# Chang-Tun-Yu/HLS-final-Visual-Odometry

Hardware: AMD Instinct MI355X
Metric: stereo frame-pairs/sec (detect+match), KITTI 1241x376; matches bit-exact (higher is better)
Workload: dtype u8; 1 GPU; KITTI 1241x376 stereo quad-match (prev/curr x L/R), default 50x50 bins; noise=0, gpu_max_hw_queues=4, streams_per_gpu=256, frames_in_hbm=8, parallelism=1x independent stream groups

## Files before the change

hls-final-visual-odometry_amd/csrc/kernels_detect.hip:

```cpp
#include "vh_dev.h"
#include "vh_wave.h"
#include <type_traits>

namespace {

__global__ void half_res_kernel(VhImages src, uint8_t *__restrict__ dst, VhGeom g) {
  const int32_t id = blockIdx.z;
  const uint8_t *__restrict__ I = vh_image_ptr(src, id);
  uint8_t *__restrict__ O = dst + (int64_t)id * g.bplm * g.Hm;
  const int32_t u = blockIdx.x * blockDim.x + threadIdx.x;
  const int32_t v = blockIdx.y;
  if (u >= g.bplm) return;
  uint32_t val = 0;
  if (u < g.Wm) {
    const int64_t r0 = (int64_t)(2 * v) * g.bpl + 2 * u, r1 = r0 + g.bpl;
    val = ((uint32_t)I[r0] + I[r0 + 1] + I[r1] + I[r1 + 1]) >> 2;
  }
  O[(int64_t)v * g.bplm + u] = (uint8_t)val;
}

__global__ void __launch_bounds__(256)
detect_nms_kernel(VhImages im, VhGeom g, uint64_t *__restrict__ rec, int32_t *__restrict__ chunk_count) {
  extern __shared__ __attribute__((aligned(16))) uint8_t smem[];
  uint8_t *sI = smem;
  int16_t *sF1 = (int16_t *)(smem + (size_t)g.IH * g.IWp);
  int16_t *sF2 = sF1 + (size_t)g.FH * g.FWp;

  const int32_t id = blockIdx.z;
  const uint8_t *__restrict__ I = vh_image_ptr(im, id);
  const int32_t n = g.n, n1 = n + 1;
  const int32_t bx0 = blockIdx.x * g.tbx, by0 = blockIdx.y * g.tby;
  const int32_t fx0 = VH_MARGIN + bx0 * n1, fy0 = VH_MARGIN + by0 * n1;
  const int32_t ix0 = fx0 - 2, iy0 = fy0 - 2;
  const int32_t tid = threadIdx.x;

  for (int32_t k = tid; k < g.IH * g.IWp; k += 256) {
    const int32_t r = k / g.IWp, c = k - r * g.IWp;
    const int32_t gx = ix0 + c, gy = iy0 + r;
    uint8_t v = 0;
    if (c < g.IW && gx < g.bplm && gy < g.Hm) v = I[(int64_t)gy * g.bplm + gx];
    sI[k] = v;
  }
  __syncthreads();

  {
    const int32_t nseg = max(1, 256 / g.FW);
    const int32_t rows_per = (g.FH + nseg - 1) / nseg;
    for (int32_t task = tid; task < g.FW * nseg; task += 256) {
      const int32_t seg = task / g.FW, cx = task - seg * g.FW;
      const int32_t r0 = seg * rows_per, r1 = min(g.FH, r0 + rows_per);
      if (r0 >= r1) continue;
      int32_t h5[5], h3[5], hc[5], cc[5];
#pragma unroll
      for (int32_t k = 0; k < 4; k++) {
        const uint8_t *p = sI + (size_t)(r0 + k) * g.IWp + cx;
        const int32_t a = p[0], b = p[1], c = p[2], d = p[3], e = p[4];
        h5[k + 1] = a + b + c + d + e; h3[k + 1] = b + c + d; hc[k + 1] = a + b - d - e; cc[k + 1] = c;
      }
      for (int32_t fr = r0; fr < r1; fr++) {
#pragma unroll
        for (int32_t k = 0; k < 4; k++) { h5[k] = h5[k + 1]; h3[k] = h3[k + 1]; hc[k] = hc[k + 1]; cc[k] = cc[k + 1]; }
        const uint8_t *p = sI + (size_t)(fr + 4) * g.IWp + cx;
        const int32_t a = p[0], b = p[1], c = p[2], d = p[3], e = p[4];
        h5[4] = a + b + c + d + e; h3[4] = b + c + d; hc[4] = a + b - d - e; cc[4] = c;
        const int32_t f2 = hc[0] + hc[1] - hc[3] - hc[4];
        const int32_t f1 = -(h5[0] + h5[1] + h5[2] + h5[3] + h5[4]) + 2 * (h3[1] + h3[2] + h3[3]) + 7 * cc[2];
        sF1[(size_t)fr * g.FWp + cx] = (int16_t)f1;
        sF2[(size_t)fr * g.FWp + cx] = (int16_t)f2;
      }
    }
  }
  __syncthreads();

  int32_t *sCnt = (int32_t *)(sF2 + (size_t)g.FH * g.FWp);
  uint32_t *sWork = (uint32_t *)(sCnt + 1);
  uint16_t *sCode = (uint16_t *)(sWork + 4 * g.tbx * g.tby);
  const int32_t nblk_tile = g.tbx * g.tby;
  if (tid == 0) *sCnt = 0;
  for (int32_t k = tid; k < 4 * nblk_tile; k += 256) sCode[k] = VH_NO_CODE;
  __syncthreads();
  const int32_t xlim = (g.Wm - 1 - VH_MARGIN) - fx0, ylim = (g.Hm - 1 - VH_MARGIN) - fy0;
  const int32_t lby = tid / g.tbx, lbx = tid - lby * g.tbx;
  const int32_t bx = bx0 + lbx, by = by0 + lby;
  const bool have_block = tid < nblk_tile && bx < g.nbx && by < g.nby;
  if (have_block) {
    const int32_t fx = n + lbx * n1, fy = n + lby * n1;
    int32_t ex[4], ey[4], ev[4];
    ex[0] = ex[1] = ex[2] = ex[3] = fx;
    ey[0] = ey[1] = ey[2] = ey[3] = fy;
    ev[0] = ev[1] = sF1[(size_t)fy * g.FWp + fx];
    ev[2] = ev[3] = sF2[(size_t)fy * g.FWp + fx];
    for (int32_t j2 = fy; j2 <= fy + n; j2++) {
      for (int32_t i2 = fx; i2 <= fx + n; i2++) {
        int32_t cur = sF1[(size_t)j2 * g.FWp + i2];
        if (cur < ev[0]) { ex[0] = i2; ey[0] = j2; ev[0] = cur; }
        else if (cur > ev[1]) { ex[1] = i2; ey[1] = j2; ev[1] = cur; }
        cur = sF2[(size_t)j2 * g.FWp + i2];
        if (cur < ev[2]) { ex[2] = i2; ey[2] = j2; ev[2] = cur; }
        else if (cur > ev[3]) { ex[3] = i2; ey[3] = j2; ev[3] = cur; }
      }
    }
#pragma unroll
    for (int32_t c = 0; c < 4; c++) {
      const bool pass = (c & 1) ? (ev[c] >= g.tau) : (ev[c] <= -g.tau);
      if (pass) sWork[atomicAdd(sCnt, 1)] = (uint32_t)ex[c] | ((uint32_t)ey[c] << 10) | ((uint32_t)c << 20) | ((uint32_t)tid << 22);
    }
  }
  __syncthreads();
  const int32_t nwork = *sCnt;
  for (int32_t w = tid; w < nwork; w += 256) {
    const uint32_t e = sWork[w];
    const int32_t cx = e & 1023, cy = (e >> 10) & 1023, c = (e >> 20) & 3, owner = e >> 22;
    const int32_t oby = owner / g.tbx, obx = owner - oby * g.tbx;
    const int32_t fx = n + obx * n1, fy = n + oby * n1;
    const int16_t *F = (c < 2) ? sF1 : sF2;
    const bool is_min = (c & 1) == 0;
    const int32_t val = F[(size_t)cy * g.FWp + cx];
    const int32_t jhi = min(cy + n, ylim), ihi = min(cx + n, xlim);
    bool ok = true;
    for (int32_t j2 = cy - n; j2 <= jhi && ok; j2++) {
      for (int32_t i2 = cx - n; i2 <= ihi; i2++) {
        const int32_t cur = F[(size_t)j2 * g.FWp + i2];
        const bool outside = (i2 < fx) | (i2 > fx + n) | (j2 < fy) | (j2 > fy + n);
        if (outside && (is_min ? (cur < val) : (cur > val))) { ok = false; break; }
      }
    }
    if (ok) sCode[owner * 4 + c] = (uint16_t)(((cy - fy) << 6) | (cx - fx));
  }
  __syncthreads();
  if (have_block) {
    uint64_t code = 0;
    int32_t cnt = 0;
#pragma unroll
    for (int32_t c = 0; c < 4; c++) {
      const uint32_t pc = sCode[tid * 4 + c];
      code |= (uint64_t)pc << (16 * c);
      cnt += pc != VH_NO_CODE ? 1 : 0;
    }
    const int32_t blk = by * g.nbx + bx;
    rec[(int64_t)id * g.nblocks + blk] = code;
    if (cnt) atomicAdd(&chunk_count[(int64_t)id * g.nchunks + blk / VH_CHUNK], cnt);
  }
}

#ifdef VH_EMIT_TIMING
__device__ unsigned long long g_emit_t[8];
extern "C" int32_t vh_debug_emit_timing(unsigned long long *out, int32_t reset) {
  if (hipMemcpyFromSymbol(out, HIP_SYMBOL(g_emit_t), sizeof(g_emit_t)) != hipSuccess) return -3;
  if (reset) { unsigned long long z[8] = {0}; z[6] = ~0ull; if (hipMemcpyToSymbol(HIP_SYMBOL(g_emit_t), z, sizeof(z)) != hipSuccess) return -3; }
  return 0;
}
#define VH_TICK_IMPL(k) do { __syncthreads(); if (t_on_) { const unsigned long long now_ = __builtin_readcyclecounter(); atomicAdd(&g_emit_t[k], now_ - t_prev_); t_prev_ = now_; if ((k) == 4) atomicMax(&g_emit_t[7], now_); } } while (0)
#define VH_TICK_INIT_IMPL const bool t_on_ = threadIdx.x == 0 && (blockIdx.x + gridDim.x * (blockIdx.y + gridDim.y * blockIdx.z)) % 61 == 0; unsigned long long t_prev_ = __builtin_readcyclecounter(); if (t_on_) { atomicAdd(&g_emit_t[5], 1ull); atomicMin(&g_emit_t[6], t_prev_); }
#endif
#if defined(VH_EMIT_TIMING) && VH_EMIT_TIMING == 2
#define VH_DTICK(k) VH_TICK_IMPL(k)
#define VH_DTICK_INIT VH_TICK_INIT_IMPL
#else
#define VH_DTICK(k) do { } while (0)
#define VH_DTICK_INIT do { } while (0)
#endif
#if defined(VH_EMIT_TIMING) && VH_EMIT_TIMING != 2
#define VH_ETICK(k) VH_TICK_IMPL(k)
#define VH_ETICK_INIT VH_TICK_INIT_IMPL
#else
#define VH_ETICK(k) do { } while (0)
#define VH_ETICK_INIT do { } while (0)
#endif

#ifdef VH_EXP_DET_STOP
#define VH_DET_STOP(k)                                                                                   \
  if (VH_EXP_DET_STOP == (k) && g.nbx > 0) {                                                              \
    const int32_t sbx = bx0 + tid % T::TBX, sby = by0 + tid / T::TBX;                                     \
    if (sbx < g.nbx && sby < g.nby) rec[(int64_t)id * g.nblocks + sby * g.nbx + sbx] = ~0ull;              \
    return;                                                                                               \
  }
#else
#define VH_DET_STOP(k) do { } while (0)
#endif

template <int N> struct DetTile {
  static constexpr int N1 = N + 1, TBX = 32, TBY = 8;
  static constexpr int FW = TBX * N1 + 2 * N, FH = TBY * N1 + 2 * N;
  static constexpr int IW = FW + 4, IH = FH + 4;
  static constexpr int OFF = (VH_MARGIN - 2) & 3;
  static constexpr int DW = ((IW + 3 + 3) / 4 + 3) / 4 * 4;
  static constexpr int IP = DW * 4;
  static constexpr int NC = DW / 4;
  static constexpr int groups(int px) { return (FW + OFF + px - 1) / px; }
  static constexpr int seg_cost(int px, int s) {
    const int rows = (FH + s - 1) / s, waves = (groups(px) * s + 63) / 64;
    const int hrow = px == 4 ? 28 : 18, vrow = px == 4 ? 26 : 13;
    return groups(px) * s > 256 || rows * (s - 1) >= FH ? (1 << 30) : 1000 * ((rows + 4) * hrow + rows * vrow) + waves;
  }
  static constexpr int best_seg(int px) {
    int b = 1;
    for (int s = 2; s <= 16; s++)
      if (seg_cost(px, s) < seg_cost(px, b)) b = s;
    return b;
  }
#ifdef VH_DET_PX
  static constexpr int PX = VH_DET_PX;
  static constexpr int SEG = VH_DET_SEG;
#else
  static constexpr int PX = seg_cost(2, best_seg(2)) < seg_cost(4, best_seg(4)) ? 2 : 4;
  static constexpr int SEG = best_seg(PX);
#endif
  static constexpr int G = groups(PX);
  static constexpr int FP = PX * G;
  static constexpr int ROWS = (FH + SEG - 1) / SEG;
  static constexpr int BIAS = 8192;
  static_assert((G - 1) * PX / 4 + 1 <= DW - 1, "a group reads the staged dword it starts in and the next one");
  static_assert(G * SEG <= 256, "one lane per (group, row segment)");
  static constexpr int LAST = FH - (SEG - 1) * ROWS;
  static_assert(LAST >= 1, "every segment has rows");
};

template <int N>
__global__ void __launch_bounds__(256)
detect_nms_fast_kernel(VhImages im, VhGeom g, uint64_t *__restrict__ rec, int32_t *__restrict__ chunk_count) {
  using T = DetTile<N>;
  constexpr int N1 = T::N1, WN = 2 * N + 1;
  VH_DET_SETPRIO();
  constexpr int X_BYTES = (T::IH * T::IP > 6144) ? T::IH * T::IP : 6144;
  __shared__ __attribute__((aligned(16))) int16_t sF1[T::FH * T::FP];
  __shared__ __attribute__((aligned(16))) int16_t sF2[T::FH * T::FP];
  __shared__ __attribute__((aligned(16))) uint8_t sX[X_BYTES];
  uint8_t *sI = sX;

  const int32_t id = blockIdx.z, tid = threadIdx.x;
  const uint8_t *__restrict__ I = vh_image_ptr(im, id);
  const int32_t bx0 = blockIdx.x * T::TBX, by0 = blockIdx.y * T::TBY;
  const int32_t fx0 = VH_MARGIN + bx0 * N1, fy0 = VH_MARGIN + by0 * N1;
  const int32_t ix0 = fx0 - 2, iy0 = fy0 - 2;
  const int32_t ax0 = ix0 - T::OFF;
  VH_DTICK_INIT;

  {
    constexpr int NLD = (T::IH * T::NC + 255) / 256;
    typedef uint32_t u32x4a4 __attribute__((ext_vector_type(4), aligned(4)));
    typedef uint32_t u32x4 __attribute__((ext_vector_type(4)));
    const uint32_t last = (uint32_t)g.Hm * (uint32_t)g.bplm - 16u;
    u32x4 stg[NLD];
#pragma unroll
    for (int32_t i = 0; i < NLD; i++) {
      const int32_t k = min(tid + 256 * i, T::IH * T::NC - 1);
      const int32_t r = k / T::NC, c = k - r * T::NC;
      stg[i] = *(const u32x4a4 *)(I + min((uint32_t)(iy0 + r) * (uint32_t)g.bplm + (uint32_t)(ax0 + 16 * c), last));
    }
    __builtin_amdgcn_sched_barrier(0);
#pragma unroll
    for (int32_t i = 0; i < NLD; i++) {
      const int32_t k = tid + 256 * i;
      if (k < T::IH * T::NC) ((u32x4 *)sI)[k] = stg[i];
    }
  }
  __syncthreads();

  VH_DTICK(0);
  VH_DET_STOP(1);
  if (tid < T::G * T::SEG) {
    constexpr int PX = T::PX, NR = PX / 2;
    const int32_t seg = tid / T::G, gq = tid - seg * T::G;
    const int32_t r0 = seg * T::ROWS;
    {
      constexpr uint32_t HB = 512u * 0x00010001u, KB = (uint32_t)T::BIAS * 0x00010001u;
      const uint32_t *p = (const uint32_t *)sI + r0 * T::DW + (gq * PX) / 4;
      const uint32_t sel0 = 0x0c010c00u + ((PX == 2 && (gq & 1)) ? 0x00020002u : 0u);
      uint32_t *o1 = (uint32_t *)sF1 + (r0 * T::FP + PX * gq) / 2, *o2 = (uint32_t *)sF2 + (r0 * T::FP + PX * gq) / 2;
      uint32_t h5[NR][5], h3[NR][5], pc[NR][4], cc[NR][5], hcp[NR], S5[NR];
#pragma unroll
      for (int32_t h = 0; h < NR; h++) S5[h] = 0u;
#pragma unroll
      for (int32_t t = 0; t < T::ROWS + 4; t++) {
        if (t - 4 < T::LAST || r0 + t - 4 < T::FH) {
          const uint32_t A = p[t * T::DW], B = p[t * T::DW + 1];
          uint32_t pk[PX + 3];
#pragma unroll
          for (int32_t k = 0; k < PX + 3; k++) pk[k] = __builtin_amdgcn_perm(B, A, sel0 + (uint32_t)k * 0x00010001u);
          uint32_t n5[NR], n3[NR], nc[NR], nz[NR];
          if (PX == 4) {
            const uint32_t a01 = pk[0] + pk[1], a23 = pk[2] + pk[3], a34 = pk[3] + pk[4], a56 = pk[5] + pk[6];
            n3[0] = a23 + pk[1];             n3[NR - 1] = a34 + pk[5];
            n5[0] = n3[0] + pk[0] + pk[4];   n5[NR - 1] = n3[NR - 1] + pk[2] + pk[6];
            nc[0] = (a01 + HB) - a34;        nc[NR - 1] = (a23 + HB) - a56;
            nz[0] = pk[2];                   nz[NR - 1] = pk[4];
          } else {
            n3[0] = pk[1] + pk[2] + pk[3];
            n5[0] = n3[0] + pk[0] + pk[4];
            nc[0] = ((pk[0] + pk[1]) + HB) - (pk[3] + pk[4]);
            nz[0] = pk[2];
          }
          uint32_t f1[NR], f2[NR];
#pragma unroll
          for (int32_t h = 0; h < NR; h++) {
            const uint32_t old5 = h5[h][0];
#pragma unroll
            for (int32_t k = 0; k < 4; k++) { h5[h][k] = h5[h][k + 1]; h3[h][k] = h3[h][k + 1]; cc[h][k] = cc[h][k + 1]; }
            h5[h][4] = n5[h]; h3[h][4] = n3[h]; cc[h][4] = nz[h];
            S5[h] += n5[h];
            if (t >= 5) S5[h] -= old5;
#pragma unroll
            for (int32_t k = 0; k < 3; k++) pc[h][k] = pc[h][k + 1];
            if (t > 0) pc[h][3] = hcp[h] + nc[h];
            hcp[h] = nc[h];
            if (t >= 4) {
              const uint32_t S3 = h3[h][1] + h3[h][2] + h3[h][3];
              f2[h] = (pc[h][0] + KB) - pc[h][3];
              f1[h] = ((S3 + S3) + (__umul24(cc[h][2], 7u) + KB)) - S5[h];
            }
          }
          if (t >= 4) {
            if (PX == 4) {
              *(uint2 *)(o1 + (t - 4) * (T::FP / 2)) = make_uint2(f1[0], f1[NR - 1]);
              *(uint2 *)(o2 + (t - 4) * (T::FP / 2)) = make_uint2(f2[0], f2[NR - 1]);
            } else {
              o1[(t - 4) * (T::FP / 2)] = f1[0];
              o2[(t - 4) * (T::FP / 2)] = f2[0];
            }
          }
        }
      }
    }
  }
  __syncthreads();
  VH_DTICK(1);
  VH_DET_STOP(2);

  const int32_t xlim = min(max((g.Wm - 1 - VH_MARGIN) - fx0, 0), T::FW - 1);
  const int32_t ylim = min(max((g.Hm - 1 - VH_MARGIN) - fy0, 0), T::FH - 1);
  const int32_t lby = tid / T::TBX, lbx = tid % T::TBX;
  const int32_t bx = bx0 + lbx, by = by0 + lby;
  const bool have_block = bx < g.nbx && by < g.nby;
  const int32_t fx = N + lbx * N1, fy = N + lby * N1;
  uint32_t *sQueue = (uint32_t *)sX;
  uint16_t *sCode = (uint16_t *)(sQueue + 1024);
  __shared__ uint32_t sQueueN;
  if (tid == 0) sQueueN = 0;
  ((uint2 *)sCode)[tid] = make_uint2(VH_NO_CODE * 0x00010001u, VH_NO_CODE * 0x00010001u);
  __syncthreads();
  {
    typedef int16_t i16x2 __attribute__((ext_vector_type(2)));
    const int32_t lane = tid & 63;
    bool cand[4];
    uint32_t ext[4];
#pragma unroll
    for (int32_t plane = 0; plane < 2; plane++) {
      const int16_t *b = (plane ? sF2 : sF1) + fy * T::FP + fx + T::OFF;
      int32_t vn, vx;
      if (N & 1) {
        const i16x2 *bw = (const i16x2 *)b;
        i16x2 mn = bw[0], mx = mn;
#pragma unroll
        for (int32_t j = 0; j < N1; j++) {
#pragma unroll
          for (int32_t d = 0; d < N1 / 2; d++) {
            if (d == 0 && j == 0) continue;
            const i16x2 w = bw[j * (T::FP / 2) + d];
            mn = __builtin_elementwise_min(mn, w);
            mx = __builtin_elementwise_max(mx, w);
          }
        }
        vn = min((int32_t)mn.x, (int32_t)mn.y);
        vx = max((int32_t)mx.x, (int32_t)mx.y);
      } else {
        vn = vx = b[0];
#pragma unroll
        for (int32_t k = 1; k < N1 * N1; k++) {
          const int32_t cur = b[(k / N1) * T::FP + k % N1];
          vn = min(vn, cur);
          vx = max(vx, cur);
        }
      }
      cand[2 * plane] = have_block && vn <= T::BIAS - g.tau;
      cand[2 * plane + 1] = have_block && vx >= T::BIAS + g.tau;
      ext[2 * plane] = (uint32_t)vn;
      ext[2 * plane + 1] = (uint32_t)vx;
    }
    uint64_t bal[4];
#pragma unroll
    for (int32_t t = 0; t < 4; t++) bal[t] = __ballot(cand[t]);
    const uint32_t n0 = (uint32_t)__popcll(bal[0]), n1 = (uint32_t)__popcll(bal[1]);
    const uint32_t add = (n0 + (uint32_t)__popcll(bal[2])) | ((n1 + (uint32_t)__popcll(bal[3])) << 16);
    if (add) {
      uint32_t base = 0;
      if (lane == 0) base = atomicAdd(&sQueueN, add);
      base = __builtin_amdgcn_readfirstlane(base);
#pragma unroll
      for (int32_t t = 0; t < 4; t++) {
        const int32_t mm = t & 1;
        const uint32_t first = ((base >> (16 * mm)) & 0xFFFFu) + (t >= 2 ? (mm ? n1 : n0) : 0u);
        const uint32_t rank = (uint32_t)vh_wave_rank(bal[t]);
        if (cand[t]) sQueue[mm * 512 + first + rank] = (uint32_t)tid | ((uint32_t)t << 8) | (ext[t] << 16);
      }
    }
  }
  __syncthreads();
  VH_DTICK(2);
  VH_DET_STOP(3);
  {
    const int32_t n0 = (int32_t)(sQueueN & 0xFFFFu), ntot = n0 + (int32_t)(sQueueN >> 16);
    const bool unclipped = xlim == T::FW - 1 && ylim == T::FH - 1;
    auto check = [&](auto kind, auto no_clip, int32_t e) {
      const uint32_t q = sQueue[e < n0 ? e : 512 + e - n0];
      const int32_t owner = q & 255, type = (q >> 8) & 3;
      const int32_t ofy = N + (owner / T::TBX) * N1, ofx = N + (owner % T::TBX) * N1;
      const int16_t *F = ((type & 2) ? sF2 : sF1) + T::OFF;
      const int32_t val = (int32_t)(q >> 16);
      const int16_t *bb = F + ofy * T::FP + ofx;
      int32_t pos = (N << 6) | N;
#pragma unroll
      for (int32_t idx = N1 * N1 - 2; idx >= 0; idx--)
        pos = bb[(idx / N1) * T::FP + idx % N1] == val ? (((idx / N1) << 6) | (idx % N1)) : pos;
      const int32_t bj = pos >> 6, bi = pos & 63;
      const int32_t cy = ofy + bj, cx = ofx + bi;
      int32_t v[WN * WN];
      if (decltype(no_clip)::value) {
        const int16_t *w = F + (cy - N) * T::FP + (cx - N);
#pragma unroll
        for (int32_t j = 0; j < WN; j++)
#pragma unroll
          for (int32_t k = 0; k < WN; k++) v[j * WN + k] = w[j * T::FP + k];
      } else {
        int32_t col[WN];
#pragma unroll
        for (int32_t k = 0; k < WN; k++) col[k] = min(cx - N + k, xlim);
#pragma unroll
        for (int32_t j = 0; j < WN; j++) {
          const int16_t *row = F + min(cy - N + j, ylim) * T::FP;
#pragma unroll
          for (int32_t k = 0; k < WN; k++) v[j * WN + k] = row[col[k]];
        }
      }
      const int32_t centre = v[N * WN + N];
      int32_t emin = centre, emax = centre;
#pragma unroll
      for (int32_t k = 0; k < WN * WN; k++) {
        if (decltype(kind)::value != 1) emin = min(emin, v[k]);
        if (decltype(kind)::value != 0) emax = max(emax, v[k]);
      }
      const int32_t ext = decltype(kind)::value == 0 ? emin : decltype(kind)::value == 1 ? emax : ((type & 1) ? emax : emin);
      if (ext == centre) sCode[owner * 4 + type] = (uint16_t)((bj << 6) | bi);
    };
    typedef std::integral_constant<int, 0> KMin;
    typedef std::integral_constant<int, 1> KMax;
    typedef std::integral_constant<int, 2> KBoth;
    for (int32_t e = tid; e < ntot; e += 256) {
      const int32_t e0 = __builtin_amdgcn_readfirstlane(e & ~63);
      if (e0 + 63 < n0) { if (unclipped) check(KMin{}, std::true_type{}, e); else check(KMin{}, std::false_type{}, e); }
      else if (e0 >= n0) { if (unclipped) check(KMax{}, std::true_type{}, e); else check(KMax{}, std::false_type{}, e); }
      else { if (unclipped) check(KBoth{}, std::true_type{}, e); else check(KBoth{}, std::false_type{}, e); }
    }
  }
  __syncthreads();
  VH_DTICK(3);
  VH_DET_STOP(4);
  uint32_t codes[4];
  {
    const uint2 cw = ((const uint2 *)sCode)[tid];
    codes[0] = cw.x & 0xFFFFu; codes[1] = cw.x >> 16; codes[2] = cw.y & 0xFFFFu; codes[3] = cw.y >> 16;
  }

  __shared__ int32_t sChunk[16];
  const int32_t chunk_lo = (by0 * g.nbx + bx0) / VH_CHUNK;
  if (tid < 16) sChunk[tid] = 0;
  __syncthreads();
  if (have_block) {
    int32_t cnt = 0;
#pragma unroll
    for (int32_t c = 0; c < 4; c++) cnt += codes[c] != VH_NO_CODE ? 1 : 0;
    const int32_t blk = by * g.nbx + bx;
    rec[(int64_t)id * g.nblocks + blk] = (uint64_t)(codes[0] | (codes[1] << 16)) | ((uint64_t)(codes[2] | (codes[3] << 16)) << 32);
    if (cnt) atomicAdd(&sChunk[blk / VH_CHUNK - chunk_lo], cnt);
  }
  __syncthreads();
  if (tid < 16 && sChunk[tid]) atomicAdd(&chunk_count[(int64_t)id * g.nchunks + chunk_lo + tid], sChunk[tid]);
  VH_DTICK(4);
}

__constant__ int8_t c_desc_dx[16] = {-3, -3, -1, -1, +3, +3, +1, +1, -1, -1, +1, +1, -5, -5, +5, +5};
__constant__ int8_t c_desc_dy[16] = {-1, +1, -1, +1, -1, +1, -1, +1, -5, +5, -5, +5, -3, +3, -3, +3};


#ifndef VH_EMIT_NF
#define VH_EMIT_NF 2
#endif
__global__ void __launch_bounds__(256)
emit_features_kernel(VhImages im, VhGeom g, const uint64_t *__restrict__ rec,
                     const int32_t *__restrict__ chunk_count, VhSets s) {
  int32_t *__restrict__ feat = s.feat;
  int32_t *__restrict__ count = s.count;
  const int32_t cap = s.cap;
  __shared__ uint32_t sList[4 * VH_CHUNK + 1];
  __shared__ int32_t sWave[4], sWaveP[4];

  const int32_t id = blockIdx.y, chunk = blockIdx.x, tid = threadIdx.x;
  const uint8_t *__restrict__ I = vh_image_ptr(im, id);
  const int32_t set = vh_image_set(im, id);
  const int32_t n1 = g.n + 1;
  VH_DET_SETPRIO();
  VH_ETICK_INIT;

  constexpr int BPL = VH_CHUNK / 256;
  uint32_t clo[BPL], chi[BPL];
  {
    const uint2 *rp = reinterpret_cast<const uint2 *>(rec) + (int64_t)id * g.nblocks;
#pragma unroll
    for (int32_t k = 0; k < BPL; k++) {
      const uint2 c = rp[min(chunk * VH_CHUNK + tid * BPL + k, g.nblocks - 1)];
      clo[k] = c.x; chi[k] = c.y;
    }
  }
  int32_t part = 0;
  for (int32_t k = tid; k < chunk; k += 256) part += chunk_count[(int64_t)id * g.nchunks + k];
  int32_t mine = 0;
#pragma unroll
  for (int32_t k = 0; k < BPL; k++) {
    if (chunk * VH_CHUNK + tid * BPL + k >= g.nblocks) clo[k] = chi[k] = ~0u;
    mine += ((clo[k] & 0xFFFFu) != VH_NO_CODE) + ((clo[k] >> 16) != VH_NO_CODE) + ((chi[k] & 0xFFFFu) != VH_NO_CODE) + ((chi[k] >> 16) != VH_NO_CODE);
  }
  part = vh_wave_sum(part);
  const int32_t incl = vh_wave_scan(mine);
  if ((tid & 63) == 63) { sWave[tid >> 6] = incl; sWaveP[tid >> 6] = part; }
  __syncthreads();
  const int32_t base = sWaveP[0] + sWaveP[1] + sWaveP[2] + sWaveP[3];
  VH_ETICK(0);
  int32_t woff = 0;
  for (int32_t w = 0; w < (tid >> 6); w++) woff += sWave[w];
  const int32_t total = sWave[0] + sWave[1] + sWave[2] + sWave[3];
  int32_t pos = woff + incl - mine;
  {
    const int32_t blk0 = chunk * VH_CHUNK + tid * BPL;
    int32_t by = blk0 / g.nbx, bx = blk0 - by * g.nbx;
    const uint32_t org = (uint32_t)(g.n + VH_MARGIN) * ((1u << 14) + 1u);
#pragma unroll
    for (int32_t k = 0; k < BPL; k++) {
      const uint32_t pxy = org + (uint32_t)(bx * n1) + ((uint32_t)(by * n1) << 14);
#pragma unroll
      for (int32_t q = 0; q < 4; q++) {
        const uint32_t w = (q < 2) ? clo[k] : chi[k];
        const uint32_t pc = (q & 1) ? (w >> 16) : (w & 0xFFFFu);
        const bool ok = pc != VH_NO_CODE;
        const uint32_t e = pxy + (pc & 63u) + ((pc >> 6) << 14) + ((uint32_t)q << 28);
        sList[ok ? pos : 4 * VH_CHUNK] = e;
        pos += ok ? 1 : 0;
      }
      if (++bx == g.nbx) { bx = 0; by++; }
    }
  }
  __syncthreads();
  if (chunk == g.nchunks - 1 && tid == 0) count[set] = base + total;
  VH_ETICK(1);
  const int32_t grp = tid >> 4, k = tid & 15;
  const int32_t dx = c_desc_dx[k], dy = c_desc_dy[k];
  constexpr int NF = VH_EMIT_NF;
  const int32_t prk = min(k, 14) - 7;
  typedef uint32_t u32x4a1 __attribute__((ext_vector_type(4), aligned(1)));
  struct Coords { int32_t fs[NF], us[NF], vs[NF], cs[NF]; bool lives[NF]; };
  auto fetch = [&](int32_t f0, Coords &q, u32x4a1 (&prow)[NF]) {
#pragma unroll
    for (int32_t h = 0; h < NF; h++) {
      q.fs[h] = f0 + 16 * h + grp;
      q.lives[h] = q.fs[h] < total;
      const uint32_t e = sList[q.lives[h] ? q.fs[h] : 0];
      q.us[h] = e & 0x3FFF; q.vs[h] = (e >> 14) & 0x3FFF; q.cs[h] = e >> 28;
#ifdef VH_EXP_NOPATCH
      prow[h] = u32x4a1{(uint32_t)q.us[h], (uint32_t)q.vs[h], 0u, 0u};
#else
      prow[h] = *(const u32x4a1 *)(I + (__umul24((uint32_t)(q.vs[h] + prk), (uint32_t)g.bplm) + (uint32_t)(q.us[h] - 7)));
#endif
    }
  };
  Coords qa, qb;
  u32x4a1 pa[NF], pb[NF];
  if (total > 0) fetch(0, qa, pa);

  constexpr int ROWS_LDS = 64;
  __shared__ int32_t sRow[4 * ROWS_LDS];
  __shared__ __attribute__((aligned(16))) uint16_t sLoc[4 * VH_CHUNK];
  const int32_t blk_first = chunk * VH_CHUNK, blk_last = min(blk_first + VH_CHUNK, g.nblocks) - 1;
  const int32_t v_first = ((blk_first / g.nbx) * n1 + g.n + VH_MARGIN) * g.scale;
  const int32_t v_span = ((blk_last / g.nbx) * n1 + g.n + VH_MARGIN + g.n) * g.scale + g.scale - v_first;
  const bool rows_in_lds = v_span <= ROWS_LDS;
  int32_t *__restrict__ rowh = s.row_hist + (int64_t)set * 4 * s.H;
  auto bin_of_entry = [&](uint32_t e) {
    const int32_t uu = (int32_t)(e & 0x3FFF) * g.scale, vv = (int32_t)((e >> 14) & 0x3FFF) * g.scale, c = e >> 28;
    const int32_t ubin = s.binsize == 1 ? uu : (int32_t)__umulhi((uint32_t)uu, s.inv_binsize);
    const int32_t vbin = s.binsize == 1 ? vv : (int32_t)__umulhi((uint32_t)vv, s.inv_binsize);
    return (c * s.ubn + min(ubin, s.ubn - 1)) * s.vbn + min(vbin, s.vbn - 1);
  };
  const bool have0 = tid < total && base + tid < cap;
  const int32_t b0 = have0 ? bin_of_entry(sList[tid]) : 0;
  int32_t slot0 = 0;
  if (have0) slot0 = atomicAdd(&s.hist[(int64_t)set * s.nbins + b0], 1);
  if (rows_in_lds) {
    for (int32_t k = tid; k < 4 * ROWS_LDS; k += 256) sRow[k] = 0;
    __syncthreads();
    for (int32_t f = tid; f < total && base + f < cap; f += 256) {
      const uint32_t e = sList[f];
      const int32_t vv = (int32_t)((e >> 14) & 0x3FFF) * g.scale, c = e >> 28;
      sLoc[f] = (uint16_t)atomicAdd(&sRow[c * ROWS_LDS + (vv - v_first)], 1);
    }
    __syncthreads();
    for (int32_t k = tid; k < 4 * ROWS_LDS; k += 256) {
      const int32_t cnt = sRow[k], c = k / ROWS_LDS, vv = v_first + k % ROWS_LDS;
      if (cnt) sRow[k] = atomicAdd(&rowh[c * s.H + vv], cnt);
    }
    __syncthreads();
  }
  VH_ETICK(2);
  for (int32_t f = tid; f < total; f += 256) {
    const int32_t fi = base + f;
    if (fi >= cap) break;
    const uint32_t e = sList[f];
    const int32_t vv = (int32_t)((e >> 14) & 0x3FFF) * g.scale, c = e >> 28;
    const int32_t b = f == tid ? b0 : bin_of_entry(e);
    const int32_t rowrel = rows_in_lds ? sRow[c * ROWS_LDS + (vv - v_first)] + (int32_t)sLoc[f] : atomicAdd(&rowh[c * s.H + vv], 1);
    const int32_t slot = f == tid ? slot0 : atomicAdd(&s.hist[(int64_t)set * s.nbins + b], 1);
#ifdef VH_CHECK
    { int32_t sl = slot; VH_CHECK_RANGE(s, 5, sl, 0, s.stage_cap); }
#endif
    if (slot < s.stage_cap) s.stage[((int64_t)set * s.nbins + b) * s.stage_cap + slot] = make_int2(fi, rowrel);
  }

  VH_ETICK(3);
  const int32_t sh = g.scale - 1;
  int32_t *__restrict__ out = feat + (int64_t)set * cap * 12;
  uint32_t *__restrict__ fuv = s.f_uv + (int64_t)set * cap;
  const int32_t gbase = (tid & 63) & ~15, j = (k >= 4) ? (k - 4) : 0;
  const uint32_t m_u = k == 0 ? ~0u : 0u, m_v = k == 1 ? ~0u : 0u, m_c = k == 3 ? ~0u : 0u, m_d = k >= 4 ? ~0u : 0u;
  static_assert(16 * NF * 16 * 16 <= (int)sizeof(sLoc), "the patches reuse sLoc");
  __syncthreads();
  uint32_t *sPatch = (uint32_t *)sLoc + grp * (NF * 64);
  const int32_t rd0 = (dy + 5) * 4 + ((dx + 5) >> 2);
  const uint32_t psel = 0x03020100u + (uint32_t)((dx + 5) & 3) * 0x01010101u;
  auto process = [&](const Coords &q, const u32x4a1 (&prow)[NF]) {
    const int32_t *fs = q.fs, *us = q.us, *vs = q.vs, *cs = q.cs;
    const bool *lives = q.lives;
    uint32_t lo[NF][5], hi[NF][5];
    uint32_t sel[NF];
#pragma unroll
    for (int32_t h = 0; h < NF; h++) sel[h] = psel;
    __builtin_amdgcn_sched_barrier(0);
#pragma unroll
    for (int32_t h = 0; h < NF; h++)
      *(uint4 *)(sPatch + (h * 16 + k) * 4) = make_uint4(prow[h].x, prow[h].y, prow[h].z, prow[h].w);
#pragma unroll
    for (int32_t h = 0; h < NF; h++)
#pragma unroll
      for (int32_t r = 0; r < 5; r++) {
        lo[h][r] = sPatch[h * 64 + rd0 + 4 * r];
        hi[h][r] = sPatch[h * 64 + rd0 + 4 * r + 1];
      }
    __builtin_amdgcn_sched_barrier(0);
#pragma unroll
    for (int32_t h = 0; h < NF; h++) {
      const int32_t u = us[h], v = vs[h];
      uint32_t du_p = 0, du_n = 0, dv_p = 0, dv_n = 0;
#pragma unroll
      for (int32_t r = 0; r < 5; r++) {
        const uint32_t w = __builtin_amdgcn_perm(hi[h][r], lo[h][r], sel[h]);
        const uint32_t w1 = __builtin_amdgcn_perm(hi[h][r], lo[h][r], sel[h] + 0x01010101u);
        const uint32_t sw = (r == 0 || r == 4) ? 1u : (r == 2 ? 6u : 4u);
        du_p = __builtin_amdgcn_udot4(w, sw * 0x00000201u, du_p, false);
        du_n = __builtin_amdgcn_udot4(w1, sw * 0x01020000u, du_n, false);
        if (r != 2) {
          const uint32_t dw = (r == 0 || r == 4) ? 1u : 2u;
          uint32_t &acc = r < 2 ? dv_p : dv_n;
          acc = __builtin_amdgcn_udot4(w, dw * 0x00060401u, acc, false);
          acc = __builtin_amdgcn_udot4(w1, dw * 0x01040000u, acc, false);
        }
      }
      const int32_t a_du = (int32_t)(du_p - du_n), a_dv = (int32_t)(dv_p - dv_n);
      const uint32_t du = (uint32_t)min(255, max(0, (a_du >> 7) + 128));
      const uint32_t dv = (uint32_t)min(255, max(0, (a_dv >> 7) + 128));
      const uint32_t pair = du | (dv << 8);
      const uint32_t plo = __shfl(pair, gbase + 2 * j), phi = __shfl(pair, gbase + 2 * j + 1);
      const uint32_t word = (((uint32_t)u << sh) & m_u) | (((uint32_t)v << sh) & m_v) | ((uint32_t)cs[h] & m_c) | ((plo | (phi << 16)) & m_d);
      const int32_t fi = base + fs[h];
      const bool okf = lives[h] && fi < cap;
      if (okf && k < 12) out[(int64_t)fi * 12 + k] = (int32_t)word;
      if (okf && k == 12) fuv[fi] = (uint32_t)(u << sh) | ((uint32_t)(v << sh) << 16);
    }
  };
  if (total > 0) {
    for (int32_t f0 = 0;; f0 += 32 * NF) {
      const bool more1 = f0 + 16 * NF < total;
      if (more1) fetch(f0 + 16 * NF, qb, pb);
      process(qa, pa);
      if (!more1) break;
      const bool more2 = f0 + 32 * NF < total;
      if (more2) fetch(f0 + 32 * NF, qa, pa);
      process(qb, pb);
      if (!more2) break;
    }
  }
  VH_ETICK(4);
}

__global__ void planes_kernel(const uint8_t *__restrict__ I, int32_t bpl, int32_t H,
                              uint8_t *__restrict__ du, uint8_t *__restrict__ dv,
                              int16_t *__restrict__ f1, int16_t *__restrict__ f2) {
  const int32_t x = blockIdx.x * blockDim.x + threadIdx.x, y = blockIdx.y;
  if (x >= bpl) return;
  const int64_t o = (int64_t)y * bpl + x;
  int32_t r_du = 0, r_dv = 0, r_f1 = 0, r_f2 = 0;
  if (x >= 2 && x <= bpl - 3 && y >= 2 && y <= H - 3) {
    int32_t a_du = 0, a_dv = 0, a_f2 = 0, s5 = 0, s3 = 0, ctr = 0;
#pragma unroll
    for (int32_t r = 0; r < 5; r++) {
      const uint8_t *p = I + (int64_t)(y + r - 2) * bpl + (x - 2);
      const int32_t a = p[0], b = p[1], c = p[2], d = p[3], e = p[4];
      const int32_t sw = (r == 0 || r == 4) ? 1 : (r == 2 ? 6 : 4);
      const int32_t dw = (r == 0) ? 1 : (r == 1 ? 2 : (r == 2 ? 0 : (r == 3 ? -2 : -1)));
      const int32_t cw = (r < 2) ? 1 : (r == 2 ? 0 : -1);
      a_du += sw * (a + 2 * b - 2 * d - e);
      a_dv += dw * (a + 4 * b + 6 * c + 4 * d + e);
      a_f2 += cw * (a + b - d - e);
      s5 += a + b + c + d + e;
      if (r >= 1 && r <= 3) s3 += b + c + d;
      if (r == 2) ctr = c;
    }
    r_du = min(255, max(0, (a_du >> 7) + 128));
    r_dv = min(255, max(0, (a_dv >> 7) + 128));
    r_f2 = a_f2;
    if (x >= 3 && y >= 3) r_f1 = -s5 + 2 * s3 + 7 * ctr;
  }
  if (du) du[o] = (uint8_t)r_du;
  if (dv) dv[o] = (uint8_t)r_dv;
  if (f1) f1[o] = (int16_t)r_f1;
  if (f2) f2[o] = (int16_t)r_f2;
}

}

static bool images_dword_aligned(const VhImages &im, const VhGeom &g) {
  return (g.bplm % 4 == 0) && (im.stride % 4 == 0) && ((uintptr_t)im.base[0] % 4 == 0) &&
         (im.ncam < 2 || (uintptr_t)im.base[1] % 4 == 0);
}

void vh_launch_half_res(const VhImages &src, uint8_t *dst, const VhGeom &g, hipStream_t st) {
  dim3 grid((g.bplm + 255) / 256, g.Hm, src.S * src.ncam);
  hipLaunchKernelGGL(half_res_kernel, grid, dim3(256), 0, st, src, dst, g);
}

void vh_launch_detect_nms(const VhImages &im, const VhGeom &g, uint64_t *rec, int32_t *chunk_count,
                          hipStream_t st) {
  if (g.nblocks <= 0) return;
  if (images_dword_aligned(im, g) && g.n >= 1 && g.n <= 4 && g.nbx <= 2048) {
    dim3 grid((g.nbx + 31) / 32, (g.nby + 7) / 8, im.S * im.ncam);
    switch (g.n) {
      case 1: hipLaunchKernelGGL(detect_nms_fast_kernel<1>, grid, dim3(256), 0, st, im, g, rec, chunk_count); break;
      case 2: hipLaunchKernelGGL(detect_nms_fast_kernel<2>, grid, dim3(256), 0, st, im, g, rec, chunk_count); break;
      case 3: hipLaunchKernelGGL(detect_nms_fast_kernel<3>, grid, dim3(256), 0, st, im, g, rec, chunk_count); break;
      default: hipLaunchKernelGGL(detect_nms_fast_kernel<4>, grid, dim3(256), 0, st, im, g, rec, chunk_count); break;
    }
    return;
  }
  dim3 grid((g.nbx + g.tbx - 1) / g.tbx, (g.nby + g.tby - 1) / g.tby, im.S * im.ncam);
  const size_t lds = (size_t)g.IH * g.IWp + 2 * (size_t)g.FH * g.FWp * sizeof(int16_t) + 4 +
                     (size_t)g.tbx * g.tby * (16 + 8);
  hipLaunchKernelGGL(detect_nms_kernel, grid, dim3(256), lds, st, im, g, rec, chunk_count);
}

void vh_launch_emit_features(const VhImages &im, const VhGeom &g, const uint64_t *rec,
                             const int32_t *chunk_count, const VhSets &s, hipStream_t st) {
  if (g.nblocks <= 0) return;
  dim3 grid(g.nchunks, im.S * im.ncam);
  hipLaunchKernelGGL(emit_features_kernel, grid, dim3(256), 0, st, im, g, rec, chunk_count, s);
}

void vh_launch_planes(const uint8_t *img, int32_t bpl, int32_t H, uint8_t *du, uint8_t *dv,
                      int16_t *f1, int16_t *f2, hipStream_t st) {
  dim3 grid((bpl + 255) / 256, H);
  hipLaunchKernelGGL(planes_kernel, grid, dim3(256), 0, st, img, bpl, H, du, dv, f1, f2);
}
```

Measured before the change: 116,100 pairs/s.

## Compute feature descriptors with int8 MFMA against a precomputed Sobel weight table

Replaces the per-lane udot4 Sobel descriptor computation, which staged patches through LDS, with 16x16x64 int8 MFMA instructions. A constexpr table of weights (sign-flipped smooth/derivative products per descriptor position) is loaded into LDS, and each wave processes 16 features per step, using DPP swaps to pack the outputs. The kernel also gains a waves_per_eu attribute. Exactness depends on the XOR-0x80 signed offset trick and the weight encoding matching the old arithmetic, and the new layout changes the output write pattern.

Result: no change. 116,400 pairs/s (median of 6 runs) (+0.3%).

```diff
diff --git a/hls-final-visual-odometry_amd/csrc/kernels_detect.hip b/hls-final-visual-odometry_amd/csrc/kernels_detect.hip
--- a/hls-final-visual-odometry_amd/csrc/kernels_detect.hip
+++ b/hls-final-visual-odometry_amd/csrc/kernels_detect.hip
@@ -478,14 +478,28 @@
   VH_DTICK(4);
 }
 
-__constant__ int8_t c_desc_dx[16] = {-3, -3, -1, -1, +3, +3, +1, +1, -1, -1, +1, +1, -5, -5, +5, +5};
-__constant__ int8_t c_desc_dy[16] = {-1, +1, -1, +1, -1, +1, -1, +1, -5, +5, -5, +5, -3, +3, -3, +3};
-
-
-#ifndef VH_EMIT_NF
-#define VH_EMIT_NF 2
-#endif
-__global__ void __launch_bounds__(256)
+constexpr int8_t c_desc_dx[16] = {-3, -3, -1, -1, +3, +3, +1, +1, -1, -1, +1, +1, -5, -5, +5, +5};
+constexpr int8_t c_desc_dy[16] = {-1, +1, -1, +1, -1, +1, -1, +1, -5, +5, -5, +5, -3, +3, -3, +3};
+
+struct DescWeights {
+  uint32_t w[4][2][64][4];
+  constexpr DescWeights() : w{} {
+    constexpr int32_t smooth[5] = {1, 4, 6, 4, 1}, deriv[5] = {1, 2, 0, -2, -1};
+    for (int32_t s = 0; s < 4; s++)
+      for (int32_t l = 0; l < 64; l++) {
+        const int32_t n = l & 15, r = 4 * s + (l >> 4) - (c_desc_dy[n] + 5);
+        for (int32_t b = 0; b < 16; b++) {
+          const int32_t c = b - (c_desc_dx[n] + 5);
+          if (r < 0 || r > 4 || c < 0 || c > 4) continue;
+          w[s][0][l][b >> 2] |= (uint32_t)(uint8_t)(smooth[r] * deriv[c]) << (8 * (b & 3));
+          w[s][1][l][b >> 2] |= (uint32_t)(uint8_t)(deriv[r] * smooth[c]) << (8 * (b & 3));
+        }
+      }
+  }
+};
+__device__ const DescWeights c_desc_w{};
+
+__global__ void __launch_bounds__(256) __attribute__((amdgpu_waves_per_eu(6, 8)))
 emit_features_kernel(VhImages im, VhGeom g, const uint64_t *__restrict__ rec,
                      const int32_t *__restrict__ chunk_count, VhSets s) {
   int32_t *__restrict__ feat = s.feat;
@@ -551,29 +565,29 @@
   __syncthreads();
   if (chunk == g.nchunks - 1 && tid == 0) count[set] = base + total;
   VH_ETICK(1);
-  const int32_t grp = tid >> 4, k = tid & 15;
-  const int32_t dx = c_desc_dx[k], dy = c_desc_dy[k];
-  constexpr int NF = VH_EMIT_NF;
-  const int32_t prk = min(k, 14) - 7;
+  const int32_t lane = tid & 63, fl = lane & 15, rg = lane >> 4;
+  const int32_t wave0 = __builtin_amdgcn_readfirstlane(tid >> 6) * 16;
+  const int32_t ntot = __builtin_amdgcn_readfirstlane(total);
   typedef uint32_t u32x4a1 __attribute__((ext_vector_type(4), aligned(1)));
-  struct Coords { int32_t fs[NF], us[NF], vs[NF], cs[NF]; bool lives[NF]; };
-  auto fetch = [&](int32_t f0, Coords &q, u32x4a1 (&prow)[NF]) {
-#pragma unroll
-    for (int32_t h = 0; h < NF; h++) {
-      q.fs[h] = f0 + 16 * h + grp;
-      q.lives[h] = q.fs[h] < total;
-      const uint32_t e = sList[q.lives[h] ? q.fs[h] : 0];
-      q.us[h] = e & 0x3FFF; q.vs[h] = (e >> 14) & 0x3FFF; q.cs[h] = e >> 28;
+  typedef int32_t i32x4 __attribute__((ext_vector_type(4)));
+  struct Coords { int32_t u, v, c; };
+  auto fetch = [&](int32_t f0, Coords &q, u32x4a1 (&prow)[4]) {
+    const int32_t f = f0 + fl;
+    const uint32_t e = sList[f < ntot ? f : 0];
+    q.u = e & 0x3FFF; q.v = (e >> 14) & 0x3FFF; q.c = e >> 28;
+#pragma unroll
+    for (int32_t ks = 0; ks < 4; ks++) {
 #ifdef VH_EXP_NOPATCH
-      prow[h] = u32x4a1{(uint32_t)q.us[h], (uint32_t)q.vs[h], 0u, 0u};
+      prow[ks] = u32x4a1{(uint32_t)q.u, (uint32_t)q.v, (uint32_t)ks, 0u};
 #else
-      prow[h] = *(const u32x4a1 *)(I + (__umul24((uint32_t)(q.vs[h] + prk), (uint32_t)g.bplm) + (uint32_t)(q.us[h] - 7)));
+      prow[ks] = *(const u32x4a1 *)(I + (__umul24((uint32_t)(q.v + min(4 * ks + rg, 14) - 7), (uint32_t)g.bplm) + (uint32_t)(q.u - 7)));
 #endif
     }
   };
   Coords qa, qb;
-  u32x4a1 pa[NF], pb[NF];
-  if (total > 0) fetch(0, qa, pa);
+  u32x4a1 pa[4], pb[4];
+  if (wave0 < ntot) fetch(wave0, qa, pa);
+  const uint4 wt0 = reinterpret_cast<const uint4 *>(c_desc_w.w)[tid], wt1 = reinterpret_cast<const uint4 *>(c_desc_w.w)[tid + 256];
 
   constexpr int ROWS_LDS = 64;
   __shared__ int32_t sRow[4 * ROWS_LDS];
@@ -627,71 +641,53 @@
   const int32_t sh = g.scale - 1;
   int32_t *__restrict__ out = feat + (int64_t)set * cap * 12;
   uint32_t *__restrict__ fuv = s.f_uv + (int64_t)set * cap;
-  const int32_t gbase = (tid & 63) & ~15, j = (k >= 4) ? (k - 4) : 0;
-  const uint32_t m_u = k == 0 ? ~0u : 0u, m_v = k == 1 ? ~0u : 0u, m_c = k == 3 ? ~0u : 0u, m_d = k >= 4 ? ~0u : 0u;
-  static_assert(16 * NF * 16 * 16 <= (int)sizeof(sLoc), "the patches reuse sLoc");
-  __syncthreads();
-  uint32_t *sPatch = (uint32_t *)sLoc + grp * (NF * 64);
-  const int32_t rd0 = (dy + 5) * 4 + ((dx + 5) >> 2);
-  const uint32_t psel = 0x03020100u + (uint32_t)((dx + 5) & 3) * 0x01010101u;
-  auto process = [&](const Coords &q, const u32x4a1 (&prow)[NF]) {
-    const int32_t *fs = q.fs, *us = q.us, *vs = q.vs, *cs = q.cs;
-    const bool *lives = q.lives;
-    uint32_t lo[NF][5], hi[NF][5];
-    uint32_t sel[NF];
-#pragma unroll
-    for (int32_t h = 0; h < NF; h++) sel[h] = psel;
-    __builtin_amdgcn_sched_barrier(0);
-#pragma unroll
-    for (int32_t h = 0; h < NF; h++)
-      *(uint4 *)(sPatch + (h * 16 + k) * 4) = make_uint4(prow[h].x, prow[h].y, prow[h].z, prow[h].w);
-#pragma unroll
-    for (int32_t h = 0; h < NF; h++)
-#pragma unroll
-      for (int32_t r = 0; r < 5; r++) {
-        lo[h][r] = sPatch[h * 64 + rd0 + 4 * r];
-        hi[h][r] = sPatch[h * 64 + rd0 + 4 * r + 1];
-      }
-    __builtin_amdgcn_sched_barrier(0);
-#pragma unroll
-    for (int32_t h = 0; h < NF; h++) {
-      const int32_t u = us[h], v = vs[h];
-      uint32_t du_p = 0, du_n = 0, dv_p = 0, dv_n = 0;
-#pragma unroll
-      for (int32_t r = 0; r < 5; r++) {
-        const uint32_t w = __builtin_amdgcn_perm(hi[h][r], lo[h][r], sel[h]);
-        const uint32_t w1 = __builtin_amdgcn_perm(hi[h][r], lo[h][r], sel[h] + 0x01010101u);
-        const uint32_t sw = (r == 0 || r == 4) ? 1u : (r == 2 ? 6u : 4u);
-        du_p = __builtin_amdgcn_udot4(w, sw * 0x00000201u, du_p, false);
-        du_n = __builtin_amdgcn_udot4(w1, sw * 0x01020000u, du_n, false);
-        if (r != 2) {
-          const uint32_t dw = (r == 0 || r == 4) ? 1u : 2u;
-          uint32_t &acc = r < 2 ? dv_p : dv_n;
-          acc = __builtin_amdgcn_udot4(w, dw * 0x00060401u, acc, false);
-          acc = __builtin_amdgcn_udot4(w1, dw * 0x01040000u, acc, false);
-        }
-      }
-      const int32_t a_du = (int32_t)(du_p - du_n), a_dv = (int32_t)(dv_p - dv_n);
-      const uint32_t du = (uint32_t)min(255, max(0, (a_du >> 7) + 128));
-      const uint32_t dv = (uint32_t)min(255, max(0, (a_dv >> 7) + 128));
-      const uint32_t pair = du | (dv << 8);
-      const uint32_t plo = __shfl(pair, gbase + 2 * j), phi = __shfl(pair, gbase + 2 * j + 1);
-      const uint32_t word = (((uint32_t)u << sh) & m_u) | (((uint32_t)v << sh) & m_v) | ((uint32_t)cs[h] & m_c) | ((plo | (phi << 16)) & m_d);
-      const int32_t fi = base + fs[h];
-      const bool okf = lives[h] && fi < cap;
-      if (okf && k < 12) out[(int64_t)fi * 12 + k] = (int32_t)word;
-      if (okf && k == 12) fuv[fi] = (uint32_t)(u << sh) | ((uint32_t)(v << sh) << 16);
-    }
+  const int32_t lim = min(ntot, cap - base);
+  static_assert(sizeof(DescWeights) <= sizeof(sLoc), "the weight table reuses sLoc");
+  __syncthreads();
+  uint4 *sW = reinterpret_cast<uint4 *>(sLoc);
+  sW[tid] = wt0; sW[tid + 256] = wt1;
+  __syncthreads();
+  const bool odd = lane & 1;
+  auto process = [&](int32_t f0, const Coords &q, const u32x4a1 (&prow)[4]) {
+    i32x4 a_du = {0, 0, 0, 0}, a_dv = {0, 0, 0, 0};
+    int32_t wl = lane;
+    asm volatile("" : "+v"(wl));
+#pragma unroll
+    for (int32_t ks = 0; ks < 4; ks++) {
+      const i32x4 a = (i32x4)prow[ks] ^ (int32_t)0x80808080;
+      const uint4 bu = sW[(2 * ks + 0) * 64 + wl], bv = sW[(2 * ks + 1) * 64 + wl];
+      a_du = __builtin_amdgcn_mfma_i32_16x16x64_i8(a, i32x4{(int32_t)bu.x, (int32_t)bu.y, (int32_t)bu.z, (int32_t)bu.w}, a_du, 0, 0, 0);
+      a_dv = __builtin_amdgcn_mfma_i32_16x16x64_i8(a, i32x4{(int32_t)bv.x, (int32_t)bv.y, (int32_t)bv.z, (int32_t)bv.w}, a_dv, 0, 0, 0);
+    }
+    uint32_t pr[4];
+#pragma unroll
+    for (int32_t i = 0; i < 4; i++) {
+      const uint32_t du = (uint32_t)min(255, max(0, (a_du[i] >> 7) + 128));
+      const uint32_t dv = (uint32_t)min(255, max(0, (a_dv[i] >> 7) + 128));
+      pr[i] = du | (dv << 8);
+    }
+    const uint32_t p01 = pr[0] | (pr[1] << 16), p23 = pr[2] | (pr[3] << 16);
+    const uint32_t q01 = (uint32_t)__builtin_amdgcn_update_dpp((int32_t)p01, (int32_t)p01, 0xB1, 0xF, 0xF, false);
+    const uint32_t q23 = (uint32_t)__builtin_amdgcn_update_dpp((int32_t)p23, (int32_t)p23, 0xB1, 0xF, 0xF, false);
+    const uint32_t ev = odd ? q23 : p01, od = odd ? p23 : q01;
+    const int32_t fd = f0 + 4 * rg + (odd ? 2 : 0), wd = 4 + (fl >> 1);
+    if (fd < lim) out[(int64_t)(base + fd) * 12 + wd] = (int32_t)((ev & 0xFFFFu) | (od << 16));
+    if (fd + 1 < lim) out[(int64_t)(base + fd + 1) * 12 + wd] = (int32_t)((ev >> 16) | (od & 0xFFFF0000u));
+    const uint32_t uu = (uint32_t)q.u << sh, vv = (uint32_t)q.v << sh;
+    const uint32_t hw = rg == 0 ? uu : (rg == 1 ? vv : (rg == 2 ? 0u : (uint32_t)q.c));
+    const int32_t fh = f0 + fl;
+    if (fh < lim) out[(int64_t)(base + fh) * 12 + rg] = (int32_t)hw;
+    if (fh < lim && rg == 0) fuv[base + fh] = uu | (vv << 16);
   };
-  if (total > 0) {
-    for (int32_t f0 = 0;; f0 += 32 * NF) {
-      const bool more1 = f0 + 16 * NF < total;
-      if (more1) fetch(f0 + 16 * NF, qb, pb);
-      process(qa, pa);
+  if (wave0 < ntot) {
+    for (int32_t f0 = wave0;; f0 += 128) {
+      const bool more1 = f0 + 64 < ntot;
+      if (more1) fetch(f0 + 64, qb, pb);
+      process(f0, qa, pa);
       if (!more1) break;
-      const bool more2 = f0 + 32 * NF < total;
-      if (more2) fetch(f0 + 32 * NF, qa, pa);
-      process(qb, pb);
+      const bool more2 = f0 + 128 < ntot;
+      if (more2) fetch(f0 + 128, qa, pa);
+      process(f0 + 64, qb, pb);
       if (!more2) break;
     }
   }
```
